# ray-project/rayfed

Hardware: AMD Instinct MI355X
Metric: cross_party_objects_per_sec (higher is better)
Workload: dtype int64; 1 GPU; model=many_tiny_tasks (2-party aggregate loop), global_batch=2576, seq_len=1, parallelism=fed2p-weak x1 lanes, transport=cpp

## Files before the change

### csrc/xfer_core.cpp

```cpp
#include <openssl/err.h>
#include <openssl/ssl.h>
#include <pybind11/functional.h>
#include <pybind11/pybind11.h>
#include <pybind11/stl.h>

#include <arpa/inet.h>
#include <netdb.h>
#include <netinet/in.h>
#include <netinet/tcp.h>
#include <sys/socket.h>
#include <sys/uio.h>
#include <unistd.h>

#include <atomic>
#include <condition_variable>
#include <cstring>
#include <deque>
#include <map>
#include <mutex>
#include <optional>
#include <stdexcept>
#include <string>
#include <thread>
#include <unordered_map>
#include <unordered_set>
#include <vector>

namespace py = pybind11;

namespace {

constexpr uint8_t kFlagDeferAck = 1;
constexpr uint8_t kFlagStripe = 2;
constexpr uint8_t kFlagPinned = 4;
constexpr const char* kPingSeqId = "ping";

extern "C" int hipHostMalloc(void** ptr, size_t size, unsigned int flags);
extern "C" int hipHostFree(void* ptr);

struct PinnedBuf {
  char* p = nullptr;
  size_t cap = 0;
  size_t len = 0;
  bool pinned = false;
  ~PinnedBuf();
};

class PinnedPool {
 public:
  static PinnedPool& inst() {
    static PinnedPool pool;
    return pool;
  }

  ~PinnedPool() {
    for (auto& [cls, bucket] : free_)
      for (auto& b : bucket) b->p = nullptr;
  }

  std::shared_ptr<PinnedBuf> acquire(size_t n) {
    size_t cls = 1ull << (64 - __builtin_clzll(std::max<size_t>(n, 1 << 16) - 1));
    {
      std::lock_guard<std::mutex> lk(mu_);
      auto& bucket = free_[cls];
      if (!bucket.empty()) {
        auto b = bucket.back();
        bucket.pop_back();
        b->len = n;
        return b;
      }
    }
    auto b = std::make_shared<PinnedBuf>();
    void* p = nullptr;
    if (hipHostMalloc(&p, cls, 0) == 0 && p) {
      b->p = (char*)p;
      b->pinned = true;
    } else {
      b->p = (char*)malloc(cls);
      if (!b->p) throw std::bad_alloc();
      b->pinned = false;
    }
    b->cap = cls;
    b->len = n;
    return b;
  }

  void release(std::shared_ptr<PinnedBuf> b) {
    std::lock_guard<std::mutex> lk(mu_);
    auto& bucket = free_[b->cap];
    size_t limit = b->cap >= (64u << 20) ? 16 : 8;
    if (bucket.size() < limit) bucket.push_back(std::move(b));
  }

 private:
  std::mutex mu_;
  std::unordered_map<size_t, std::vector<std::shared_ptr<PinnedBuf>>> free_;
};

PinnedBuf::~PinnedBuf() {
  if (!p) return;
  if (pinned)
    hipHostFree(p);
  else
    free(p);
}

static void write_all(int fd, const char* data, size_t n) {
  while (n) {
    ssize_t w = ::send(fd, data, n, MSG_NOSIGNAL);
    if (w < 0) {
      if (errno == EINTR) continue;
      throw std::runtime_error(std::string("send: ") + strerror(errno));
    }
    data += w;
    n -= (size_t)w;
  }
}

static void writev_all(int fd, std::vector<iovec> iov) {
  size_t idx = 0;
  while (idx < iov.size()) {
    ssize_t w = ::writev(fd, iov.data() + idx, (int)(iov.size() - idx));
    if (w < 0) {
      if (errno == EINTR) continue;
      throw std::runtime_error(std::string("writev: ") + strerror(errno));
    }
    size_t ww = (size_t)w;
    while (idx < iov.size() && ww >= iov[idx].iov_len) {
      ww -= iov[idx].iov_len;
      ++idx;
    }
    if (idx < iov.size() && ww) {
      iov[idx].iov_base = (char*)iov[idx].iov_base + ww;
      iov[idx].iov_len -= ww;
    }
  }
}

static bool read_all(int fd, char* data, size_t n) {
  while (n) {
    ssize_t r = ::recv(fd, data, n, 0);
    if (r < 0) {
      if (errno == EINTR) continue;
      return false;
    }
    if (r == 0) return false;
    data += r;
    n -= (size_t)r;
  }
  return true;
}

static void set_sock_opts(int fd) {
  int one = 1;
  setsockopt(fd, IPPROTO_TCP, TCP_NODELAY, &one, sizeof(one));
  int buf = 8 << 20;
  setsockopt(fd, SOL_SOCKET, SO_SNDBUF, &buf, sizeof(buf));
  setsockopt(fd, SOL_SOCKET, SO_RCVBUF, &buf, sizeof(buf));
}

static int spin_us() {
  static int v = [] {
    const char* e = getenv("RAYFED_SPIN_US");
    return e ? atoi(e) : 120;
  }();
  return v;
}

static std::string ssl_err() {
  char buf[256];
  ERR_error_string_n(ERR_get_error(), buf, sizeof(buf));
  return std::string(buf);
}

struct Stream {
  int fd = -1;
  SSL* ssl = nullptr;

  bool read_all(char* data, size_t n) {
    if (!ssl) return ::read_all(fd, data, n);
    while (n) {
      int r = SSL_read(ssl, data, (int)std::min(n, (size_t)1 << 20));
      if (r <= 0) return false;
      data += r;
      n -= (size_t)r;
    }
    return true;
// ... 23 lines not shown
      ::close(fd);
      fd = -1;
    }
  }
};

static SSL_CTX* make_server_ctx(const std::string& cert, const std::string& key,
                                const std::string& ca) {
  SSL_CTX* ctx = SSL_CTX_new(TLS_server_method());
  if (!ctx) throw std::runtime_error("SSL_CTX_new failed");
  SSL_CTX_set_min_proto_version(ctx, TLS1_2_VERSION);
  if (SSL_CTX_use_certificate_chain_file(ctx, cert.c_str()) != 1 ||
      SSL_CTX_use_PrivateKey_file(ctx, key.c_str(), SSL_FILETYPE_PEM) != 1) {
    SSL_CTX_free(ctx);
    throw std::runtime_error("server cert/key load failed: " + ssl_err());
  }
  if (!ca.empty()) {
    if (SSL_CTX_load_verify_locations(ctx, ca.c_str(), nullptr) != 1) {
      SSL_CTX_free(ctx);
      throw std::runtime_error("server CA load failed: " + ssl_err());
    }
    SSL_CTX_set_verify(
        ctx, SSL_VERIFY_PEER | SSL_VERIFY_FAIL_IF_NO_PEER_CERT, nullptr);
  }
  return ctx;
}

static SSL_CTX* make_client_ctx(const std::string& ca, const std::string& cert,
                                const std::string& key) {
  SSL_CTX* ctx = SSL_CTX_new(TLS_client_method());
  if (!ctx) throw std::runtime_error("SSL_CTX_new failed");
  SSL_CTX_set_min_proto_version(ctx, TLS1_2_VERSION);
  if (!ca.empty() && SSL_CTX_load_verify_locations(ctx, ca.c_str(), nullptr) != 1) {
    SSL_CTX_free(ctx);
    throw std::runtime_error("client CA load failed: " + ssl_err());
  }
  SSL_CTX_set_verify(ctx, SSL_VERIFY_PEER, nullptr);
  if (!cert.empty() && !key.empty()) {
    if (SSL_CTX_use_certificate_chain_file(ctx, cert.c_str()) != 1 ||
        SSL_CTX_use_PrivateKey_file(ctx, key.c_str(), SSL_FILETYPE_PEM) != 1) {
      SSL_CTX_free(ctx);
      throw std::runtime_error("client cert/key load failed: " + ssl_err());
    }
  }
  return ctx;
}

class BodyView {
 public:
  explicit BodyView(std::shared_ptr<PinnedBuf> b) : buf_(std::move(b)) {}
  ~BodyView() {
    if (buf_) {
      try {
        PinnedPool::inst().release(std::move(buf_));
      } catch (...) {
      }
    }
  }
  char* data() const { return buf_->p; }
  size_t size() const { return buf_->len; }
  bool pinned() const { return buf_->pinned; }

 private:
  std::shared_ptr<PinnedBuf> buf_;
};

class XferServer {
 public:
  XferServer(int port, std::string job_name, std::string tls_cert = "",
             std::string tls_key = "", std::string tls_ca = "")
      : job_(std::move(job_name)), port_(port) {
    if (!tls_cert.empty()) {
      ssl_ctx_ = make_server_ctx(tls_cert, tls_key, tls_ca);
    }
  }

  ~XferServer() {
    stop();
    if (ssl_ctx_) SSL_CTX_free(ssl_ctx_);
  }

  void start(py::object consume_cb) {
    consume_cb_ = std::move(consume_cb);
    listen_fd_ = ::socket(AF_INET, SOCK_STREAM, 0);
    if (listen_fd_ < 0) throw std::runtime_error("socket() failed");
    int zero = 0, one = 1;
    setsockopt(listen_fd_, SOL_SOCKET, SO_REUSEPORT, &zero, sizeof(zero));
    setsockopt(listen_fd_, SOL_SOCKET, SO_REUSEADDR, &one, sizeof(one));
    sockaddr_in addr{};
    addr.sin_family = AF_INET;
    addr.sin_addr.s_addr = htonl(INADDR_ANY);
    addr.sin_port = htons((uint16_t)port_);
    if (bind(listen_fd_, (sockaddr*)&addr, sizeof(addr)) != 0) {
      ::close(listen_fd_);
      listen_fd_ = -1;
      throw std::runtime_error("bind failed: port in use");
    }
    if (listen(listen_fd_, 64) != 0) {
      ::close(listen_fd_);
      listen_fd_ = -1;
      throw std::runtime_error("listen failed");
    }
    running_ = true;
    accept_thread_ = std::thread([this] { accept_loop(); });
  }

  void stop() {
    bool expected = true;
    if (!running_.compare_exchange_strong(expected, false)) return;
    ::shutdown(listen_fd_, SHUT_RDWR);
    ::close(listen_fd_);
    {
      std::lock_guard<std::mutex> lk(conn_mu_);
      for (auto& c : conns_) ::shutdown(c->st.fd, SHUT_RDWR);
    }
    if (accept_thread_.joinable()) accept_thread_.join();
    {
      std::lock_guard<std::mutex> lk(conn_mu_);
      for (auto& t : conn_threads_)
        if (t.joinable()) t.join();
      conn_threads_.clear();
    }
    {
      std::lock_guard<std::mutex> lk(tok_mu_);
      tokens_.clear();
    }
    std::lock_guard<std::mutex> lk(mail_mu_);
    stopped_ = true;
    pinned_mail_.clear();
    mail_cv_.notify_all();
  }

  void complete(uint64_t token, int code, const std::string& result) {
    std::shared_ptr<SrvConn> conn;
    uint64_t req_id = 0;
    {
      std::lock_guard<std::mutex> lk(tok_mu_);
      auto it = tokens_.find(token);
      if (it == tokens_.end()) return;
      conn = it->second.first;
      req_id = it->second.second;
      tokens_.erase(it);
    }
    if (!conn->alive.load()) return;
    try {
      write_ack(*conn, req_id, (uint16_t)code, result);
    } catch (...) {
      conn->alive = false;
      ::shutdown(conn->st.fd, SHUT_RDWR);
    }
  }

  py::bytes get_data(const std::string& up, const std::string& down,
                     double timeout_s) {
    std::string key = up + '\x00' + down;
    std::string body;
    {
      py::gil_scoped_release release;
      auto deadline = std::chrono::steady_clock::now() +
                      std::chrono::duration<double>(timeout_s);
      const auto spin_until = std::chrono::steady_clock::now() +
                              std::chrono::microseconds(spin_us());
      bool got = false;
      while (!got && std::chrono::steady_clock::now() < spin_until) {
        {
          std::unique_lock<std::mutex> lk(mail_mu_, std::try_to_lock);
          if (lk.owns_lock()) {
            auto it = mail_.find(key);
            if (it != mail_.end()) {
              body = std::move(it->second);
              mail_.erase(it);
              got = true;
              break;
            }
            if (stopped_) throw std::runtime_error("server stopped");
          }
        }
        for (int i = 0; i < 32; ++i) __builtin_ia32_pause();
      }
      if (!got) {
        std::unique_lock<std::mutex> lk(mail_mu_);
        while (true) {
          auto it = mail_.find(key);
          if (it != mail_.end()) {
            body = std::move(it->second);
            mail_.erase(it);
            break;
          }
          if (stopped_) throw std::runtime_error("server stopped");
          if (mail_cv_.wait_until(lk, deadline) == std::cv_status::timeout)
            throw std::runtime_error("get_data timeout");
        }
      }
    }
    return py::bytes(body);
  }

  void post(const std::string& up, const std::string& down,
            const std::string& body) {
    std::lock_guard<std::mutex> lk(mail_mu_);
    mail_[up + '\x00' + down] = body;
    mail_cv_.notify_all();
  }

  py::object wait_view(const std::string& up, const std::string& down,
                       double timeout_s) {
    std::string key = up + '\x00' + down;
    std::shared_ptr<PinnedBuf> b;
    {
      py::gil_scoped_release release;
      std::unique_lock<std::mutex> lk(mail_mu_);
      auto deadline = std::chrono::steady_clock::now() +
                      std::chrono::duration<double>(timeout_s);
      while (true) {
        auto it = pinned_mail_.find(key);
        if (it != pinned_mail_.end()) {
          b = std::move(it->second);
          pinned_mail_.erase(it);
          break;
        }
        if (stopped_) throw std::runtime_error("server stopped");
        if (mail_cv_.wait_until(lk, deadline) == std::cv_status::timeout)
          throw std::runtime_error("wait_view timeout");
      }
    }
    return py::cast(new BodyView(std::move(b)),
                    py::return_value_policy::take_ownership);
  }

  py::object try_view(const std::string& up, const std::string& down) {
    std::string key = up + '\x00' + down;
    std::shared_ptr<PinnedBuf> b;
    {
      std::lock_guard<std::mutex> lk(mail_mu_);
      auto it = pinned_mail_.find(key);
      if (it == pinned_mail_.end()) return py::none();
      b = std::move(it->second);
      pinned_mail_.erase(it);
    }
    return py::cast(new BodyView(std::move(b)),
                    py::return_value_policy::take_ownership);
  }

  std::optional<py::bytes> try_take(const std::string& up,
                                    const std::string& down) {
    std::string key = up + '\x00' + down;
    std::string body;
    {
      py::gil_scoped_release release;
      std::lock_guard<std::mutex> lk(mail_mu_);
      auto it = mail_.find(key);
      if (it == mail_.end()) return std::nullopt;
      body = std::move(it->second);
      mail_.erase(it);
    }
    return py::bytes(body);
  }

  uint64_t received_op_count() const { return recv_count_.load(); }

 private:
  struct SrvConn {
    Stream st;
    std::mutex write_mu;
    std::atomic<bool> alive{true};
  };

  struct Assembly {
    std::string data;
    std::shared_ptr<PinnedBuf> pbuf;
    std::atomic<uint64_t> got{0};
    uint64_t total;
    uint32_t cnt;
    std::unique_ptr<std::atomic<uint8_t>[]> seen;
    Assembly(uint64_t t, uint32_t c, bool pinned)
        : total(t), cnt(c), seen(new std::atomic<uint8_t>[c]) {
      for (uint32_t i = 0; i < c; ++i) seen[i].store(0);
      if (pinned)
        pbuf = PinnedPool::inst().acquire(t);
      else
        data.resize(t);
    }
    char* base() { return pbuf ? pbuf->p : data.data(); }
  };

  static bool drain(Stream& st, uint64_t n) {
    char scratch[65536];
    while (n) {
      size_t k = (size_t)std::min<uint64_t>(n, sizeof(scratch));
      if (!st.read_all(scratch, k)) return false;
      n -= k;
    }
    return true;
  }

  static void write_ack(SrvConn& c, uint64_t req_id, uint16_t code,
                        const std::string& result) {
    char ack[14];
    uint32_t ack_len = 10 + (uint32_t)result.size();
    memcpy(ack, &ack_len, 4);
    memcpy(ack + 4, &req_id, 8);
    memcpy(ack + 12, &code, 2);
    std::lock_guard<std::mutex> lk(c.write_mu);
    if (!c.alive.load()) throw std::runtime_error("connection closed");
    c.st.write_all(ack, 14);
    if (!result.empty()) c.st.write_all(result.data(), result.size());
  }

  void accept_loop() {
    while (running_) {
      int fd = ::accept(listen_fd_, nullptr, nullptr);
      if (fd < 0) {
        if (running_ && errno == EINTR) continue;
        break;
      }
      set_sock_opts(fd);
      auto conn = std::make_shared<SrvConn>();
      conn->st.fd = fd;
      std::lock_guard<std::mutex> lk(conn_mu_);
      conns_.push_back(conn);
      conn_threads_.emplace_back([this, conn] { conn_loop(conn); });
    }
  }

  void conn_loop(std::shared_ptr<SrvConn> conn) {
    Stream& st = conn->st;
    if (ssl_ctx_) {
      st.ssl = SSL_new(ssl_ctx_);
      SSL_set_fd(st.ssl, st.fd);
      if (SSL_accept(st.ssl) != 1) {
        conn->alive = false;
        st.close_free();
        return;
      }
    }
    std::vector<char> buf;
    while (running_) {
      char head[16];
      if (!st.read_all(head, 16)) break;
      uint64_t total, req_id;
      memcpy(&total, head, 8);
      memcpy(&req_id, head + 8, 8);
      if (total < 12 || total > (64ull << 30)) break;
      char meta[4];
      if (!st.read_all(meta, 4)) break;
      const uint8_t flags = (uint8_t)meta[0];
      const uint8_t job_len = (uint8_t)meta[1];
      const uint8_t up_len = (uint8_t)meta[2];
      const uint8_t down_len = (uint8_t)meta[3];
      const size_t names_len = (size_t)job_len + up_len + down_len;
      const size_t fixed =
          8 + 4 + names_len + ((flags & kFlagStripe) ? 24u : 0u);
      if (total < fixed) break;
      char names[768];
      if (!st.read_all(names, names_len)) break;
      std::string job(names, job_len);
      std::string up(names + job_len, up_len);
      std::string down(names + job_len + up_len, down_len);
      const uint64_t payload_len = total - fixed;

      uint16_t code = 200;
      std::string result = "OK";
      if (flags & kFlagStripe) {
        char smeta[24];
        if (!st.read_all(smeta, 24)) break;
        uint32_t idx, cnt;
        uint64_t s_off, body_total;
        memcpy(&idx, smeta, 4);
        memcpy(&cnt, smeta + 4, 4);
        memcpy(&s_off, smeta + 8, 8);
        memcpy(&body_total, smeta + 16, 8);
        if (cnt == 0 || idx >= cnt || body_total > (64ull << 30) ||
            s_off + payload_len > body_total)
          break;
        if (job != job_) {
          if (!drain(st, payload_len)) break;
          code = 417;
          result = "JobName mis-match: expected " + job_ + ", got " + job;
        } else {
          std::string key = up + '\x00' + down;
          const bool pinned = (flags & kFlagPinned) != 0;
          std::shared_ptr<Assembly> asmb;
          bool tombstoned = false;
          {
            std::lock_guard<std::mutex> lk(asm_mu_);
            auto& slot = asm_[key];
            if (!slot) {
              if (delivered_set_.count(key)) {
                asm_.erase(key);
                tombstoned = true;
              } else {
                slot = std::make_shared<Assembly>(body_total, cnt, pinned);
              }
            } else if (slot->total != body_total || slot->cnt != cnt) {
              slot = std::make_shared<Assembly>(body_total, cnt, pinned);
            }
            if (!tombstoned) asmb = slot;
          }
          if (tombstoned || asmb->seen[idx].exchange(1)) {
            if (!drain(st, payload_len)) break;
          } else
          if (!st.read_all(asmb->base() + s_off, payload_len)) {
            asmb->seen[idx].store(0);
            break;
          } else if (asmb->got.fetch_add(payload_len) + payload_len ==
                     body_total) {
            {
              std::lock_guard<std::mutex> lk(asm_mu_);
              asm_.erase(key);
              delivered_set_.insert(key);
              delivered_fifo_.push_back(key);
              if (delivered_fifo_.size() > 256) {
                delivered_set_.erase(delivered_fifo_.front());
                delivered_fifo_.pop_front();
              }
            }
            recv_count_.fetch_add(1);
            std::lock_guard<std::mutex> lk(mail_mu_);
            if (asmb->pbuf)
              pinned_mail_[key] = std::move(asmb->pbuf);
            else
              mail_[key] = std::move(asmb->data);
            mail_cv_.notify_all();
          }
        }
        try {
          write_ack(*conn, req_id, code, result);
        } catch (...) {
          break;
        }
        continue;
      }
      buf.resize(payload_len);
      if (!st.read_all(buf.data(), payload_len)) break;
      size_t off = 0;

      if (job != job_) {
        code = 417;
        result = "JobName mis-match: expected " + job_ + ", got " + job;
      } else if (up == kPingSeqId && down == kPingSeqId) {
      } else if (flags & kFlagDeferAck) {
        uint64_t token = next_token_.fetch_add(1);
        {
          std::lock_guard<std::mutex> lk(tok_mu_);
          tokens_[token] = {conn, req_id};
        }
        bool handed_off = false;
        {
          py::gil_scoped_acquire gil;
          try {
            py::bytes body(buf.data() + off, buf.size() - off);
            consume_cb_(up, down, body, token);
            handed_off = true;
          } catch (const std::exception& e) {
            code = 500;
            result = std::string("consume dispatch failed: ") + e.what();
          }
        }
        if (handed_off) continue;
        std::lock_guard<std::mutex> lk(tok_mu_);
        tokens_.erase(token);
      } else {
        recv_count_.fetch_add(1);
        std::lock_guard<std::mutex> lk(mail_mu_);
        mail_[up + '\x00' + down] =
            std::string(buf.data() + off, buf.size() - off);
        mail_cv_.notify_all();
      }

      try {
        write_ack(*conn, req_id, code, result);
      } catch (...) {
        break;
      }
    }
    {
      std::lock_guard<std::mutex> lk(conn->write_mu);
      conn->alive = false;
      st.close_free();
    }
  }

  std::string job_;
  int port_;
  int listen_fd_ = -1;
  std::atomic<bool> running_{false};
  bool stopped_ = false;
  std::thread accept_thread_;
  std::mutex conn_mu_;
  std::vector<std::shared_ptr<SrvConn>> conns_;
  std::vector<std::thread> conn_threads_;
  std::mutex mail_mu_;
  std::condition_variable mail_cv_;
  std::map<std::string, std::string> mail_;
  std::mutex asm_mu_;
  std::unordered_map<std::string, std::shared_ptr<Assembly>> asm_;
  std::unordered_set<std::string> delivered_set_;
  std::deque<std::string> delivered_fifo_;
  std::unordered_map<std::string, std::shared_ptr<PinnedBuf>> pinned_mail_;
  std::atomic<uint64_t> recv_count_{0};
  std::mutex tok_mu_;
  std::unordered_map<uint64_t, std::pair<std::shared_ptr<SrvConn>, uint64_t>>
      tokens_;
  std::atomic<uint64_t> next_token_{1};
  py::object consume_cb_;
  SSL_CTX* ssl_ctx_ = nullptr;
};

class XferClient {
 public:
  XferClient(std::string job_name, std::string tls_ca = "",
             std::string tls_cert = "", std::string tls_key = "",
             std::string server_name = "")
      : job_(std::move(job_name)), server_name_(std::move(server_name)) {
    if (!tls_ca.empty() || !tls_cert.empty()) {
      ssl_ctx_ = make_client_ctx(tls_ca, tls_cert, tls_key);
    }
  }
  ~XferClient() {
    close_all();
    if (ssl_ctx_) SSL_CTX_free(ssl_ctx_);
  }

  static std::vector<std::pair<const char*, size_t>> slice_views(
      const std::vector<std::pair<const char*, size_t>>& views, uint64_t lo,
      uint64_t hi) {
    std::vector<std::pair<const char*, size_t>> out;
    uint64_t pos = 0;
    for (const auto& v : views) {
      uint64_t vlo = pos, vhi = pos + v.second;
      pos = vhi;
      if (vhi <= lo || vlo >= hi) continue;
      uint64_t s = std::max(vlo, lo), e = std::min(vhi, hi);
      out.emplace_back(v.first + (s - vlo), (size_t)(e - s));
    }
    return out;
  }

  int send_striped(const std::string& host, int port, const std::string& up,
                   const std::string& down,
                   const std::vector<std::pair<const char*, size_t>>& views,
                   uint64_t body_len, int stripes, double timeout_s,
                   std::string* result_out, bool pinned = false) {
    std::string names;
    names.push_back((char)(kFlagStripe | (pinned ? kFlagPinned : 0)));
    names.push_back((char)job_.size());
    names.push_back((char)up.size());
    names.push_back((char)down.size());
    names += job_;
    names += up;
    names += down;
    const uint64_t chunk = (body_len + stripes - 1) / stripes;
    std::vector<int> codes((size_t)stripes, 0);
    std::vector<std::string> results((size_t)stripes);
    std::vector<std::string> errs((size_t)stripes);
    std::vector<std::thread> threads;
    for (int i = 0; i < stripes; ++i) {
      threads.emplace_back([&, i] {
        try {
          const uint64_t lo = (uint64_t)i * chunk;
          const uint64_t hi = std::min(body_len, lo + chunk);
          auto sub = slice_views(views, lo, hi);
          char smeta[24];
          uint32_t idx = (uint32_t)i, cnt = (uint32_t)stripes;
          memcpy(smeta, &idx, 4);
          memcpy(smeta + 4, &cnt, 4);
          memcpy(smeta + 8, &lo, 8);
          memcpy(smeta + 16, &body_len, 8);
          uint64_t total = 8 + names.size() + 24 + (hi - lo);
          if (ssl_ctx_) {
            codes[i] = stripe_tls(host, port, names, smeta, sub, total,
                                  timeout_s, &results[i]);
            return;
          }
          std::shared_ptr<Conn> conn_sp = get_conn(host, port, i + 1);
          Conn& conn = *conn_sp;
          std::shared_ptr<Pending> pending = std::make_shared<Pending>();
          uint64_t req_id;
          {
            std::lock_guard<std::mutex> lk(conn.write_mu);
            req_id = conn.next_id++;
            {
              std::lock_guard<std::mutex> lk2(conn.pend_mu);
              conn.pending[req_id] = pending;
            }
            char head[16];
            memcpy(head, &total, 8);
            memcpy(head + 8, &req_id, 8);
            std::vector<iovec> iov;
            iov.push_back({head, 16});
            iov.push_back({(void*)names.data(), names.size()});
            iov.push_back({smeta, 24});
            for (auto& v : sub) iov.push_back({(void*)v.first, v.second});
            try {
              writev_all(conn.fd, std::move(iov));
            } catch (...) {
              conn.alive = false;
              throw;
            }
          }
          std::unique_lock<std::mutex> lk(pending->mu);
          auto deadline = std::chrono::steady_clock::now() +
                          std::chrono::duration<double>(timeout_s);
          while (!pending->done) {
            if (pending->cv.wait_until(lk, deadline) ==
                std::cv_status::timeout)
              throw std::runtime_error("stripe ack timeout");
          }
          if (pending->broken)
            throw std::runtime_error("connection broken awaiting stripe ack");
          codes[i] = pending->code;
          results[i] = pending->result;
        } catch (const std::exception& e) {
          errs[i] = e.what();
        }
      });
    }
    for (auto& t : threads) t.join();
    for (int i = 0; i < stripes; ++i)
      if (!errs[i].empty())
        throw std::runtime_error("stripe " + std::to_string(i) +
                                 " failed: " + errs[i]);
    for (int i = 0; i < stripes; ++i) {
      if (codes[i] != 200) {
        if (result_out) *result_out = results[i];
        return codes[i];
      }
    }
    if (result_out) *result_out = "OK";
    return 200;
  }

  int stripe_tls(const std::string& host, int port, const std::string& names,
                 const char* smeta,
                 const std::vector<std::pair<const char*, size_t>>& sub,
                 uint64_t total, double timeout_s, std::string* result_out) {
    std::string key = host + ":" + std::to_string(port);
    std::unique_ptr<Stream> st = acquire_tls_conn(key, host, port);
    set_recv_timeout(st->fd, std::max(1.0, timeout_s));
    uint64_t req_id = tls_req_id_.fetch_add(1);
    try {
      char head[16];
      memcpy(head, &total, 8);
      memcpy(head + 8, &req_id, 8);
      std::vector<iovec> iov;
      iov.push_back({head, 16});
      iov.push_back({(void*)names.data(), names.size()});
      iov.push_back({(void*)smeta, 24});
      for (auto& v : sub) iov.push_back({(void*)v.first, v.second});
      st->write_iov(std::move(iov));
      char ahead[14];
      if (!st->read_all(ahead, 14))
        throw std::runtime_error("connection broken awaiting stripe ack");
      uint32_t len;
      uint64_t rid;
      uint16_t code;
      memcpy(&len, ahead, 4);
      memcpy(&rid, ahead + 4, 8);
      memcpy(&code, ahead + 12, 2);
      std::string result;
      if (len > 10) {
        result.resize(len - 10);
        if (!st->read_all(result.data(), result.size()))
          throw std::runtime_error("connection broken reading stripe ack");
      }
      if (rid != req_id)
        throw std::runtime_error("ack id mismatch on TLS stripe");
      release_tls_conn(key, std::move(st));
      if (result_out) *result_out = result;
      return code;
    } catch (...) {
      st->close_free();
      throw;
    }
  }

  int send(const std::string& host, int port, const std::string& up,
           const std::string& down, std::vector<py::buffer> parts,
           bool defer_ack, double timeout_s, std::string* result_out,
           int stripes = 1, bool pinned = false) {
    std::vector<std::pair<const char*, size_t>> views;
    views.reserve(parts.size());
    size_t body_len = 0;
    std::vector<py::buffer_info> infos;
    infos.reserve(parts.size());
    for (auto& b : parts) {
      infos.emplace_back(b.request());
      auto& info = infos.back();
      views.emplace_back((const char*)info.ptr,
                         (size_t)(info.size * info.itemsize));
      body_len += views.back().second;
    }

    if (stripes > 1 && !defer_ack && body_len > 0) {
      py::gil_scoped_release release;
      return send_striped(host, port, up, down, views, body_len, stripes,
                          timeout_s, result_out, pinned);
    }

    uint8_t flags = defer_ack ? kFlagDeferAck : 0;
    std::string preamble;
    preamble.push_back((char)flags);
    preamble.push_back((char)job_.size());
    preamble.push_back((char)up.size());
    preamble.push_back((char)down.size());
    preamble += job_;
    preamble += up;
    preamble += down;

    uint64_t total = 8  + preamble.size() + body_len;

    int code;
    std::string result;
// ... 247 lines not shown
    std::unordered_map<std::string, std::shared_ptr<Conn>> conns;
    {
      std::lock_guard<std::mutex> lk(conns_mu_);
      conns.swap(conns_);
    }
    for (auto& [key, conn] : conns) {
      ::shutdown(conn->fd, SHUT_RDWR);
      if (conn->reader.joinable()) conn->reader.join();
      ::close(conn->fd);
    }
    std::lock_guard<std::mutex> lk2(tls_mu_);
    for (auto& [key, pool] : tls_pool_)
      for (auto& st : pool) st->close_free();
    tls_pool_.clear();
  }

 private:
  struct Pending {
    std::mutex mu;
    std::condition_variable cv;
    std::atomic<bool> done{false};
    bool broken = false;
    uint16_t code = 0;
    std::string result;
  };

  struct Conn {
    int fd = -1;
    uint64_t next_id = 1;
    std::mutex write_mu;
    std::mutex pend_mu;
    std::unordered_map<uint64_t, std::shared_ptr<Pending>> pending;
    std::thread reader;
    std::atomic<bool> alive{true};
  };

  std::shared_ptr<Conn> get_conn(const std::string& host, int port,
                                 int slot = 0) {
    std::string key = host + ":" + std::to_string(port);
    if (slot) key += "#" + std::to_string(slot);
    std::lock_guard<std::mutex> lk(conns_mu_);
    auto it = conns_.find(key);
    if (it != conns_.end() && it->second->alive) return it->second;
    int fd = ::socket(AF_INET, SOCK_STREAM, 0);
    if (fd < 0) throw std::runtime_error("socket() failed");
    sockaddr_in addr{};
    addr.sin_family = AF_INET;
    addr.sin_port = htons((uint16_t)port);
    if (inet_pton(AF_INET, host.c_str(), &addr.sin_addr) != 1) {
      hostent* he = gethostbyname(host.c_str());
      if (!he) {
        ::close(fd);
        throw std::runtime_error("resolve failed: " + host);
      }
      memcpy(&addr.sin_addr, he->h_addr, sizeof(addr.sin_addr));
    }
    if (connect(fd, (sockaddr*)&addr, sizeof(addr)) != 0) {
      ::close(fd);
      throw std::runtime_error(std::string("connect failed: ") +
                               strerror(errno));
    }
    set_sock_opts(fd);
    auto conn = std::make_shared<Conn>();
    conn->fd = fd;
    std::shared_ptr<Conn> sp = conn;
    conn->reader = std::thread([this, sp] { reader_loop(sp.get()); });
    auto& entry = conns_[key];
    if (entry) {
      ::shutdown(entry->fd, SHUT_RDWR);
      if (entry->reader.joinable()) entry->reader.detach();
      dead_.push_back(entry);
    }
    entry = conn;
    return conn;
  }

  void reader_loop(Conn* conn) {
    while (true) {
      char head[14];
      if (!read_all(conn->fd, head, 14)) break;
      uint32_t len;
      uint64_t req_id;
      uint16_t code;
      memcpy(&len, head, 4);
      memcpy(&req_id, head + 4, 8);
      memcpy(&code, head + 12, 2);
      std::string result;
      if (len > 10) {
        result.resize(len - 10);
        if (!read_all(conn->fd, result.data(), result.size())) break;
      }
      std::shared_ptr<Pending> p;
      {
        std::lock_guard<std::mutex> lk(conn->pend_mu);
        auto it = conn->pending.find(req_id);
        if (it != conn->pending.end()) {
          p = it->second;
          conn->pending.erase(it);
        }
      }
      if (p) {
        std::lock_guard<std::mutex> lk(p->mu);
        p->done = true;
        p->code = code;
        p->result = std::move(result);
        p->cv.notify_all();
      }
    }
    conn->alive = false;
    std::lock_guard<std::mutex> lk(conn->pend_mu);
    for (auto& [id, p] : conn->pending) {
      std::lock_guard<std::mutex> lk2(p->mu);
      p->done = true;
      p->broken = true;
      p->cv.notify_all();
    }
    conn->pending.clear();
  }

  std::string job_;
  std::string server_name_;
  SSL_CTX* ssl_ctx_ = nullptr;
  std::mutex conns_mu_;
  std::unordered_map<std::string, std::shared_ptr<Conn>> conns_;
  std::vector<std::shared_ptr<Conn>> dead_;
  std::mutex tls_mu_;
  std::unordered_map<std::string, std::vector<std::unique_ptr<Stream>>> tls_pool_;
  std::atomic<uint64_t> tls_req_id_{1};
  std::mutex async_mu_;
  std::unordered_map<uint64_t, std::shared_ptr<Pending>> async_;
  std::atomic<uint64_t> async_id_{1};
};

}

PYBIND11_MODULE(_xfer, m) {
  m.doc() = "rayfed_amd C++ transport core (plaintext cross-silo hot path)";
  py::class_<BodyView>(m, "BodyView", py::buffer_protocol())
      .def_buffer([](BodyView& v) {
        return py::buffer_info(v.data(), sizeof(uint8_t),
                               py::format_descriptor<uint8_t>::format(), 1,
                               {v.size()}, {sizeof(uint8_t)});
      })
      .def("__len__", &BodyView::size)
      .def_property_readonly("pinned", &BodyView::pinned);
  py::class_<XferServer>(m, "XferServer")
      .def(py::init<int, std::string, std::string, std::string, std::string>(),
           py::arg("port"), py::arg("job_name"), py::arg("tls_cert") = "",
           py::arg("tls_key") = "", py::arg("tls_ca") = "")
      .def("start", &XferServer::start, py::arg("consume_cb"))
      .def("stop", &XferServer::stop,
           py::call_guard<py::gil_scoped_release>())
      .def("get_data", &XferServer::get_data, py::arg("up"), py::arg("down"),
           py::arg("timeout_s") = 600.0)
      .def("complete", &XferServer::complete, py::arg("token"),
           py::arg("code"), py::arg("result") = std::string(),
           py::call_guard<py::gil_scoped_release>())
      .def("post", &XferServer::post, py::call_guard<py::gil_scoped_release>())
      .def("wait_view", &XferServer::wait_view, py::arg("up"),
           py::arg("down"), py::arg("timeout_s") = 60.0)
      .def("try_view", &XferServer::try_view)
      .def("try_take", &XferServer::try_take)
      .def_property_readonly("received_op_count",
                             &XferServer::received_op_count);
  py::class_<XferClient>(m, "XferClient")
      .def(py::init<std::string, std::string, std::string, std::string,
                    std::string>(),
           py::arg("job_name"), py::arg("tls_ca") = "",
           py::arg("tls_cert") = "", py::arg("tls_key") = "",
           py::arg("server_name") = "")
      .def(
          "send",
          [](XferClient& c, const std::string& host, int port,
             const std::string& up, const std::string& down,
             std::vector<py::buffer> parts, bool defer_ack,
             double timeout_s, int stripes, bool pinned) {
            std::string result;
            int code =
                c.send(host, port, up, down, std::move(parts), defer_ack,
                       timeout_s, &result, stripes, pinned);
            return py::make_tuple(code, result);
          },
          py::arg("host"), py::arg("port"), py::arg("up"), py::arg("down"),
          py::arg("parts"), py::arg("defer_ack") = false,
          py::arg("timeout_s") = 60.0, py::arg("stripes") = 1,
          py::arg("pinned") = false)
      .def("send_async", &XferClient::send_async, py::arg("host"),
           py::arg("port"), py::arg("up"), py::arg("down"), py::arg("parts"),
           py::arg("defer_ack") = false)
      .def("wait_ack", &XferClient::wait_ack, py::arg("handle"),
           py::arg("timeout_s") = 60.0,
           py::call_guard<py::gil_scoped_release>())
      .def("close_all", &XferClient::close_all,
           py::call_guard<py::gil_scoped_release>());
}
```

### rayfed_amd/proxy/xfer.py

```python
from __future__ import annotations

import logging
import threading
import time
from concurrent.futures import Future, ThreadPoolExecutor
from concurrent.futures import TimeoutError as FutureTimeoutError
from typing import Dict, Optional

from rayfed_amd import config as fed_config
from rayfed_amd.ops import tensor_codec
from rayfed_amd.proxy.grpc import frames
from rayfed_amd.runtime.object_ref import ObjectRef

logger = logging.getLogger(__name__)

_OBJ_MARKER = b"\x00RFOBJ"


def _load_xfer():
    import torch

    import rayfed_amd._xfer as xfer

    return xfer
# ... 558 lines not shown
        self.gpu_plane = None
        self._stats_lock = threading.Lock()
        self.receive_op_count = 0
        self._deferred_count = 0

    @property
    def proxy(self):
        return self

    @property
    def received_op_count(self) -> int:
        return int(self._server.received_op_count) + self._deferred_count

    def _consume_deferred(self, up: str, down: str, body: bytes, token: int):
        self._consume_pool.submit(self._consume_one, up, down, body, token)

    def _consume_one(self, up: str, down: str, body: bytes, token: int):
        try:
            kind, header, payload = frames.decode_frame(body)
            obj = tensor_codec.decode(
                {k: header[k] for k in ("skel", "tensors", "ipc_group")
                 if k in header},
                memoryview(payload),
                self.gpu_plane,
                self._allowed_list,
                allow_lazy=True,
            )
        except Exception as e:
            logger.warning("xfer deferred consume failed: %r", e)
            self._server.complete(token, 500, f"consume failed: {e!r}")
            return
        lazies = (
            self.gpu_plane.pop_pending_lazies()
            if self.gpu_plane is not None
            else []
        )
        with self._objs_lock:
            self._objs[(up, down)] = obj
            self._deferred_count += 1
        self._server.post(up, down, _OBJ_MARKER)
        if not lazies:
            self._server.complete(token, 200)
            return
        remaining = [len(lazies)]
        lock = threading.Lock()

        def _one_done():
            with lock:
                remaining[0] -= 1
                done = remaining[0] == 0
            if done:
                self._server.complete(token, 200)

        for lz in lazies:
            lz._attach_completer(_one_done)

    def _take(self, up: str, down: str, body: bytes):
        if bytes(body) == _OBJ_MARKER:
            with self._objs_lock:
                return self._objs.pop((up, down))
        kind, header, payload = frames.decode_frame(body)
        from rayfed_amd._private import serialization

        if kind == frames.KIND_ERROR:
            raise serialization.loads(payload, self._allowed_list)
        if kind == frames.KIND_TENSOR:
            return tensor_codec.decode(
                header, memoryview(payload), self.gpu_plane, self._allowed_list
            )
        if kind == frames.KIND_CHUNKED:
            _ik, inner_header, _ = frames.decode_frame(payload)
            return tensor_codec.decode_streamed(
                inner_header, header["xlen"], header["xc"],
                self._iter_chunks(up, down, header["xk"]),
                self.gpu_plane, self._allowed_list,
            )
        return serialization.loads(payload, self._allowed_list)

    def _iter_chunks(self, up: str, down: str, k: int):
        import time as _time

        remaining = set(range(k))
        deadline = _time.monotonic() + 600
        while remaining:
            got = None
            for i in sorted(remaining):
                b = self._server.try_view(f"{up}\x01x{i}", down)
                if b is not None:
                    got = (i, b)
                    break
            if got is None:
                err = self._server.try_take(up, down)
                if err is not None:
                    self._take(up, down, err)
                    raise RuntimeError(
                        "unexpected non-error frame during chunked receive"
                    )
                if _time.monotonic() > deadline:
                    raise TimeoutError("chunk-streamed receive stalled")
                i = min(remaining)
                try:
                    b = self._server.wait_view(f"{up}\x01x{i}", down, 0.25)
                    got = (i, b)
                except RuntimeError as e:
                    if "timeout" in str(e):
                        continue
                    raise
            remaining.discard(got[0])
            if _xfer_debug():
                import sys as _sys

                print(f"[xfer-rx] chunk {got[0]} ({len(got[1])>>20}MiB) "
                      f"t={_time.monotonic():.3f}",
                      file=_sys.stderr, flush=True)
            yield got

    def get_data(self, src_party, upstream_seq_id, curr_seq_id) -> Future:
        up, down = str(upstream_seq_id), str(curr_seq_id)
        with self._stats_lock:
            self.receive_op_count += 1
        body = self._server.try_take(up, down)
        if body is not None:
            fut: Future = Future()
            try:
                fut.set_result(self._take(up, down, body))
            except BaseException as e:
                fut.set_exception(e)
            return fut

        def _wait(timeout=None):
            deadline = None if timeout is None else time.monotonic() + timeout
            while True:
                if deadline is None:
                    chunk = 60.0
                else:
                    chunk = min(60.0, deadline - time.monotonic())
                    if chunk <= 0:
                        raise FutureTimeoutError()
                try:
                    b = self._server.get_data(up, down, chunk)
                    break
                except RuntimeError as e:
                    if "timeout" in str(e):
                        continue
                    raise
            return self._take(up, down, b)

        return _LazyFuture(_wait)

    def _get_stats(self) -> Dict[str, int]:
        return {"receive_op_count": self.receive_op_count}

    def stop(self):
        self._server.stop()
        self._pool.shutdown(wait=False, cancel_futures=True)
        self._consume_pool.shutdown(wait=False, cancel_futures=True)


class _LazyFuture(Future):

    def __init__(self, fetch):
        super().__init__()
        self._fetch = fetch
        self._claim = threading.Lock()

    def result(self, timeout=None):
        if not self.done() and self._claim.acquire(blocking=False):
            try:
                if not self.done():
                    try:
                        value = self._fetch(timeout)
                    except FutureTimeoutError:
                        raise
                    except BaseException as e:
                        self.set_exception(e)
                    else:
                        self.set_result(value)
            finally:
                self._claim.release()
        return super().result(timeout)

    def exception(self, timeout=None):
        if not self.done():
            try:
                self.result(timeout)
            except BaseException:
                pass
        return super().exception(timeout)
```

### setup.py

```python
import os

from setuptools import find_packages, setup

os.environ.setdefault("PYTORCH_ROCM_ARCH", "gfx950")

from torch.utils import cpp_extension

setup(
    name="rayfed_amd",
    version="0.2.0",
    packages=find_packages(include=["rayfed_amd", "rayfed_amd.*"]),
    ext_modules=[
        cpp_extension.CUDAExtension(
            name="rayfed_amd._hip",
            sources=["csrc/rayfed_hip.hip"],
            include_dirs=[os.path.abspath("csrc")],
            extra_compile_args={
                "cxx": ["-O3", "-std=c++17"],
                "nvcc": ["-O3", "-std=c++17"],
            },
        ),
        cpp_extension.CppExtension(
            name="rayfed_amd._xfer",
            sources=["csrc/xfer_core.cpp"],
            extra_compile_args=["-O3", "-std=c++17", "-pthread"],
            libraries=["ssl", "crypto", "amdhip64"],
            library_dirs=["/opt/rocm/lib"],
            include_dirs=["/opt/rocm/include"],
        ),
    ],
    cmdclass={"build_ext": cpp_extension.BuildExtension},
)
```

Measured before the change: 15220 objects/s.

## Let spinning receivers pump small frames directly from connection sockets

While get_data spins waiting for a message, the waiting thread now peeks each plain (non-TLS) connection socket and consumes small unflagged frames itself, delivering its own payload directly and posting others to the mailbox. This removes the cross-thread handoff from the connection thread to the waiter through the mutex and condition variable. Connection threads now poll and take a per-connection rx mutex so the two readers never interleave on one socket. Acks are also coalesced into a single write, and stripe chunking is guarded for small bodies. The change adds locking complexity and extra recv syscalls per spin iteration.

```diff
diff --git a/csrc/xfer_core.cpp b/csrc/xfer_core.cpp
--- a/csrc/xfer_core.cpp
+++ b/csrc/xfer_core.cpp
@@ -8,6 +8,7 @@
 #include <netdb.h>
 #include <netinet/in.h>
 #include <netinet/tcp.h>
+#include <poll.h>
 #include <sys/socket.h>
 #include <sys/uio.h>
 #include <unistd.h>
@@ -26,13 +27,15 @@
 #include <unordered_set>
 #include <vector>
 
+#include "xfer_rx.h"
+
 namespace py = pybind11;
 
 namespace {
 
-constexpr uint8_t kFlagDeferAck = 1;
-constexpr uint8_t kFlagStripe = 2;
-constexpr uint8_t kFlagPinned = 4;
+using xfer_rx::kFlagDeferAck;
+using xfer_rx::kFlagStripe;
+using xfer_rx::kFlagPinned;
 constexpr const char* kPingSeqId = "ping";
 
 extern "C" int hipHostMalloc(void** ptr, size_t size, unsigned int flags);
@@ -362,16 +365,25 @@
   }
 
   py::bytes get_data(const std::string& up, const std::string& down,
-                     double timeout_s) {
+                     double timeout_s, int spin_us_arg = -1) {
     std::string key = up + '\x00' + down;
     std::string body;
     {
       py::gil_scoped_release release;
-      auto deadline = std::chrono::steady_clock::now() +
-                      std::chrono::duration<double>(timeout_s);
-      const auto spin_until = std::chrono::steady_clock::now() +
-                              std::chrono::microseconds(spin_us());
+      const auto start = std::chrono::steady_clock::now();
+      auto deadline = start + std::chrono::duration<double>(timeout_s);
+      const int spin = spin_us_arg < 0 ? spin_us() : spin_us_arg;
+      const auto spin_until =
+          std::min<std::chrono::steady_clock::time_point>(
+              start + std::chrono::microseconds(spin),
+              std::chrono::time_point_cast<
+                  std::chrono::steady_clock::duration>(deadline));
       bool got = false;
+      const bool pump = spin > 0 && !ssl_ctx_;
+      std::vector<std::shared_ptr<SrvConn>> snap;
+      std::vector<uint8_t> backoff;
+      uint64_t snap_gen = 0;
+      bool have_snap = false;
       while (!got && std::chrono::steady_clock::now() < spin_until) {
         {
           std::unique_lock<std::mutex> lk(mail_mu_, std::try_to_lock);
@@ -386,10 +398,36 @@
             if (stopped_) throw std::runtime_error("server stopped");
           }
         }
+        if (pump) {
+          const uint64_t gen = conn_gen_.load(std::memory_order_acquire);
+          if (!have_snap || gen != snap_gen) {
+            snap.clear();
+            std::lock_guard<std::mutex> lk(conn_mu_);
+            snap_gen = conn_gen_.load(std::memory_order_acquire);
+            for (auto& c : conns_)
+              if (c->alive.load()) snap.push_back(c);
+            backoff.assign(snap.size(), 0);
+            have_snap = true;
+          }
+          for (size_t ci = 0; ci < snap.size(); ++ci) {
+            if (backoff[ci]) {
+              --backoff[ci];
+              continue;
+            }
+            bool left = false;
+            if (pump_conn(*snap[ci], key, &body, &left)) {
+              got = true;
+              break;
+            }
+            if (left) backoff[ci] = 64;
+          }
+          if (got) break;
+        }
         for (int i = 0; i < 32; ++i) __builtin_ia32_pause();
       }
       if (!got) {
         std::unique_lock<std::mutex> lk(mail_mu_);
+        bool parked = false;
         while (true) {
           auto it = mail_.find(key);
           if (it != mail_.end()) {
@@ -398,6 +436,10 @@
             break;
           }
           if (stopped_) throw std::runtime_error("server stopped");
+          if (!parked) {
+            parked = true;
+            rx_parked_.fetch_add(1, std::memory_order_relaxed);
+          }
           if (mail_cv_.wait_until(lk, deadline) == std::cv_status::timeout)
             throw std::runtime_error("get_data timeout");
         }
@@ -469,9 +511,18 @@
 
   uint64_t received_op_count() const { return recv_count_.load(); }
 
+  py::dict rx_stats() const {
+    py::dict d;
+    d["waiter"] = rx_waiter_.load();
+    d["conn"] = rx_conn_.load();
+    d["parked"] = rx_parked_.load();
+    return d;
+  }
+
  private:
   struct SrvConn {
     Stream st;
+    std::mutex rx_mu;
     std::mutex write_mu;
     std::atomic<bool> alive{true};
   };
@@ -511,10 +562,65 @@
     memcpy(ack, &ack_len, 4);
     memcpy(ack + 4, &req_id, 8);
     memcpy(ack + 12, &code, 2);
+    char small[14 + 64];
+    std::string big;
+    char* out = small;
+    if (result.size() > sizeof(small) - 14) {
+      big.resize(14 + result.size());
+      out = big.data();
+    }
+    memcpy(out, ack, 14);
+    memcpy(out + 14, result.data(), result.size());
     std::lock_guard<std::mutex> lk(c.write_mu);
     if (!c.alive.load()) throw std::runtime_error("connection closed");
-    c.st.write_all(ack, 14);
-    if (!result.empty()) c.st.write_all(result.data(), result.size());
+    c.st.write_all(out, 14 + result.size());
+  }
+
+  bool pump_conn(SrvConn& c, const std::string& want_key,
+                 std::string* body_out, bool* left) {
+    if (!c.alive.load(std::memory_order_relaxed)) return false;
+    char buf[xfer_rx::kSmallFrameMax];
+    xfer_rx::Preamble pre;
+    {
+      std::unique_lock<std::mutex> rx(c.rx_mu, std::try_to_lock);
+      if (!rx.owns_lock() || !c.alive.load()) return false;
+      const xfer_rx::Took took =
+          xfer_rx::take_small_frame(c.st.fd, job_, buf, sizeof(buf), &pre);
+      if (took != xfer_rx::Took::kFrame) {
+        *left = took == xfer_rx::Took::kLeft;
+        return false;
+      }
+    }
+    const char* names = buf + xfer_rx::Preamble::names_off();
+    std::string key;
+    key.reserve((size_t)pre.up_len + 1 + pre.down_len);
+    key.append(names + pre.job_len, pre.up_len);
+    key.push_back('\x00');
+    key.append(names + pre.job_len + pre.up_len, pre.down_len);
+    const char* body = buf + pre.body_off();
+    const size_t body_len = (size_t)pre.payload_len;
+    bool mine = false;
+    if (pre.up_len == 4 && pre.down_len == 4 &&
+        memcmp(names + pre.job_len, "pingping", 8) == 0) {
+    } else {
+      recv_count_.fetch_add(1);
+      rx_waiter_.fetch_add(1, std::memory_order_relaxed);
+      if (key == want_key) {
+        body_out->assign(body, body_len);
+        mine = true;
+      } else {
+        std::lock_guard<std::mutex> lk(mail_mu_);
+        mail_[key] = std::string(body, body_len);
+        mail_cv_.notify_all();
+      }
+    }
+    try {
+      write_ack(c, pre.req_id, 200, "OK");
+    } catch (...) {
+      std::lock_guard<std::mutex> rx(c.rx_mu);
+      if (c.alive.load()) ::shutdown(c.st.fd, SHUT_RDWR);
+    }
+    return mine;
   }
 
   void accept_loop() {
@@ -530,6 +636,7 @@
       std::lock_guard<std::mutex> lk(conn_mu_);
       conns_.push_back(conn);
       conn_threads_.emplace_back([this, conn] { conn_loop(conn); });
+      conn_gen_.fetch_add(1, std::memory_order_release);
     }
   }
 
@@ -544,30 +651,39 @@
         return;
       }
     }
+    const bool plain = st.ssl == nullptr;
     std::vector<char> buf;
     while (running_) {
-      char head[16];
-      if (!st.read_all(head, 16)) break;
-      uint64_t total, req_id;
-      memcpy(&total, head, 8);
-      memcpy(&req_id, head + 8, 8);
-      if (total < 12 || total > (64ull << 30)) break;
-      char meta[4];
-      if (!st.read_all(meta, 4)) break;
-      const uint8_t flags = (uint8_t)meta[0];
-      const uint8_t job_len = (uint8_t)meta[1];
-      const uint8_t up_len = (uint8_t)meta[2];
-      const uint8_t down_len = (uint8_t)meta[3];
-      const size_t names_len = (size_t)job_len + up_len + down_len;
-      const size_t fixed =
-          8 + 4 + names_len + ((flags & kFlagStripe) ? 24u : 0u);
-      if (total < fixed) break;
-      char names[768];
-      if (!st.read_all(names, names_len)) break;
-      std::string job(names, job_len);
-      std::string up(names + job_len, up_len);
-      std::string down(names + job_len + up_len, down_len);
-      const uint64_t payload_len = total - fixed;
+      char hm[xfer_rx::kHeadMetaLen];
+      std::unique_lock<std::mutex> rx(conn->rx_mu, std::defer_lock);
+      if (plain) {
+        pollfd pfd{st.fd, POLLIN, 0};
+        int pr = ::poll(&pfd, 1, 500);
+        if (pr < 0 && errno != EINTR) break;
+        if (pr <= 0) continue;
+        rx.lock();
+        ssize_t r = ::recv(st.fd, hm, sizeof(hm), MSG_DONTWAIT);
+        if (r < 0) {
+          if (errno == EAGAIN || errno == EWOULDBLOCK || errno == EINTR)
+            continue;
+          break;
+        }
+        if (r == 0) break;
+        if ((size_t)r < sizeof(hm) &&
+            !st.read_all(hm + r, sizeof(hm) - (size_t)r))
+          break;
+      } else {
+        if (!st.read_all(hm, sizeof(hm))) break;
+      }
+      xfer_rx::Preamble pre;
+      if (!xfer_rx::parse_head_meta(hm, &pre)) break;
+      const uint64_t req_id = pre.req_id;
+      const uint8_t flags = pre.flags;
+      char names[xfer_rx::kMaxNamesLen];
+      if (!st.read_all(names, pre.names_len)) break;
+      std::string job, up, down;
+      xfer_rx::split_names(pre, names, &job, &up, &down);
+      const uint64_t payload_len = pre.payload_len;
 
       uint16_t code = 200;
       std::string result = "OK";
@@ -626,6 +742,7 @@
               }
             }
             recv_count_.fetch_add(1);
+            rx_conn_.fetch_add(1, std::memory_order_relaxed);
             std::lock_guard<std::mutex> lk(mail_mu_);
             if (asmb->pbuf)
               pinned_mail_[key] = std::move(asmb->pbuf);
@@ -634,6 +751,7 @@
             mail_cv_.notify_all();
           }
         }
+        if (rx.owns_lock()) rx.unlock();
         try {
           write_ack(*conn, req_id, code, result);
         } catch (...) {
@@ -656,6 +774,7 @@
           tokens_[token] = {conn, req_id};
         }
         bool handed_off = false;
+        if (rx.owns_lock()) rx.unlock();
         {
           py::gil_scoped_acquire gil;
           try {
@@ -672,12 +791,14 @@
         tokens_.erase(token);
       } else {
         recv_count_.fetch_add(1);
+        rx_conn_.fetch_add(1, std::memory_order_relaxed);
         std::lock_guard<std::mutex> lk(mail_mu_);
         mail_[up + '\x00' + down] =
             std::string(buf.data() + off, buf.size() - off);
         mail_cv_.notify_all();
       }
 
+      if (rx.owns_lock()) rx.unlock();
       try {
         write_ack(*conn, req_id, code, result);
       } catch (...) {
@@ -685,6 +806,7 @@
       }
     }
     {
+      std::lock_guard<std::mutex> rxl(conn->rx_mu);
       std::lock_guard<std::mutex> lk(conn->write_mu);
       conn->alive = false;
       st.close_free();
@@ -709,6 +831,10 @@
   std::deque<std::string> delivered_fifo_;
   std::unordered_map<std::string, std::shared_ptr<PinnedBuf>> pinned_mail_;
   std::atomic<uint64_t> recv_count_{0};
+  std::atomic<uint64_t> conn_gen_{0};
+  std::atomic<uint64_t> rx_waiter_{0};
+  std::atomic<uint64_t> rx_conn_{0};
+  std::atomic<uint64_t> rx_parked_{0};
   std::mutex tok_mu_;
   std::unordered_map<uint64_t, std::pair<std::shared_ptr<SrvConn>, uint64_t>>
       tokens_;
@@ -760,7 +886,9 @@
     names += job_;
     names += up;
     names += down;
-    const uint64_t chunk = (body_len + stripes - 1) / stripes;
+    const uint64_t chunk =
+        std::max<uint64_t>(1, (body_len + stripes - 1) / stripes);
+    stripes = (int)std::max<uint64_t>(1, (body_len + chunk - 1) / chunk);
     std::vector<int> codes((size_t)stripes, 0);
     std::vector<std::string> results((size_t)stripes);
     std::vector<std::string> errs((size_t)stripes);
@@ -768,7 +896,7 @@
     for (int i = 0; i < stripes; ++i) {
       threads.emplace_back([&, i] {
         try {
-          const uint64_t lo = (uint64_t)i * chunk;
+          const uint64_t lo = std::min(body_len, (uint64_t)i * chunk);
           const uint64_t hi = std::min(body_len, lo + chunk);
           auto sub = slice_views(views, lo, hi);
           char smeta[24];
@@ -1322,7 +1450,7 @@
       .def("stop", &XferServer::stop,
            py::call_guard<py::gil_scoped_release>())
       .def("get_data", &XferServer::get_data, py::arg("up"), py::arg("down"),
-           py::arg("timeout_s") = 600.0)
+           py::arg("timeout_s") = 600.0, py::arg("spin_us") = -1)
       .def("complete", &XferServer::complete, py::arg("token"),
            py::arg("code"), py::arg("result") = std::string(),
            py::call_guard<py::gil_scoped_release>())
@@ -1332,7 +1460,8 @@
       .def("try_view", &XferServer::try_view)
       .def("try_take", &XferServer::try_take)
       .def_property_readonly("received_op_count",
-                             &XferServer::received_op_count);
+                             &XferServer::received_op_count)
+      .def_property_readonly("rx_stats", &XferServer::rx_stats);
   py::class_<XferClient>(m, "XferClient")
       .def(py::init<std::string, std::string, std::string, std::string,
                     std::string>(),
diff --git a/csrc/xfer_rx.h b/csrc/xfer_rx.h
--- /dev/null
+++ b/csrc/xfer_rx.h
@@ -0,0 +1,125 @@
+#pragma once
+
+#include <sys/socket.h>
+#include <sys/types.h>
+
+#include <cerrno>
+#include <cstdint>
+#include <cstring>
+#include <string>
+
+namespace xfer_rx {
+
+constexpr uint8_t kFlagDeferAck = 1;
+constexpr uint8_t kFlagStripe = 2;
+constexpr uint8_t kFlagPinned = 4;
+
+constexpr size_t kHeadLen = 16;
+constexpr size_t kMetaLen = 4;
+constexpr size_t kHeadMetaLen = kHeadLen + kMetaLen;
+constexpr size_t kStripeMetaLen = 24;
+constexpr size_t kMaxNamesLen = 3 * 255;
+constexpr uint64_t kMaxTotal = 64ull << 30;
+constexpr size_t kSmallFrameMax = 64 * 1024;
+
+struct Preamble {
+  uint64_t total = 0;
+  uint64_t req_id = 0;
+  uint8_t flags = 0;
+  uint8_t job_len = 0;
+  uint8_t up_len = 0;
+  uint8_t down_len = 0;
+  size_t names_len = 0;
+  size_t fixed = 0;
+  uint64_t payload_len = 0;
+
+  uint64_t frame_len() const { return kHeadLen + (total - 8); }
+  static constexpr size_t names_off() { return kHeadMetaLen; }
+  size_t body_off() const { return kHeadMetaLen + names_len; }
+};
+
+inline bool parse_head_meta(const char* p, Preamble* out) {
+  Preamble pre;
+  memcpy(&pre.total, p, 8);
+  memcpy(&pre.req_id, p + 8, 8);
+  if (pre.total < 12 || pre.total > kMaxTotal) return false;
+  pre.flags = (uint8_t)p[16];
+  pre.job_len = (uint8_t)p[17];
+  pre.up_len = (uint8_t)p[18];
+  pre.down_len = (uint8_t)p[19];
+  pre.names_len = (size_t)pre.job_len + pre.up_len + pre.down_len;
+  pre.fixed = 8 + kMetaLen + pre.names_len +
+              ((pre.flags & kFlagStripe) ? kStripeMetaLen : 0u);
+  if (pre.total < pre.fixed) return false;
+  pre.payload_len = pre.total - pre.fixed;
+  *out = pre;
+  return true;
+}
+
+inline void split_names(const Preamble& pre, const char* names,
+                        std::string* job, std::string* up,
+                        std::string* down) {
+  job->assign(names, pre.job_len);
+  up->assign(names + pre.job_len, pre.up_len);
+  down->assign(names + pre.job_len + pre.up_len, pre.down_len);
+}
+
+enum class Peeked {
+  kIncomplete,
+  kPlainSmall,
+  kLeave,
+  kBad,
+};
+
+inline Peeked classify_peeked(const char* buf, size_t n,
+                              const std::string& job, Preamble* out) {
+  if (n < kHeadMetaLen) return Peeked::kIncomplete;
+  Preamble pre;
+  if (!parse_head_meta(buf, &pre)) return Peeked::kBad;
+  if (pre.flags != 0) return Peeked::kLeave;
+  if (pre.frame_len() > kSmallFrameMax) return Peeked::kLeave;
+  if (n < pre.frame_len()) return Peeked::kIncomplete;
+  if (pre.job_len != job.size() ||
+      memcmp(buf + Preamble::names_off(), job.data(), job.size()) != 0)
+    return Peeked::kLeave;
+  *out = pre;
+  return Peeked::kPlainSmall;
+}
+
+enum class Took {
+  kEmpty,
+  kFrame,
+  kIncomplete,
+  kLeft,
+};
+
+inline Took take_small_frame(int fd, const std::string& job, char* buf,
+                             size_t cap, Preamble* out) {
+  if (cap > kSmallFrameMax) cap = kSmallFrameMax;
+  ssize_t r;
+  do {
+    r = ::recv(fd, buf, cap, MSG_PEEK | MSG_DONTWAIT);
+  } while (r < 0 && errno == EINTR);
+  if (r < 0 && (errno == EAGAIN || errno == EWOULDBLOCK)) return Took::kEmpty;
+  if (r <= 0) return Took::kLeft;
+  Preamble pre;
+  switch (classify_peeked(buf, (size_t)r, job, &pre)) {
+    case Peeked::kPlainSmall:
+      break;
+    case Peeked::kIncomplete:
+      return (size_t)r >= cap ? Took::kLeft : Took::kIncomplete;
+    default:
+      return Took::kLeft;
+  }
+  size_t want = (size_t)pre.frame_len(), have = 0;
+  while (have < want) {
+    ssize_t t = ::recv(fd, buf + have, want - have, MSG_DONTWAIT);
+    if (t < 0 && errno == EINTR) continue;
+    if (t <= 0) return Took::kLeft;
+    have += (size_t)t;
+  }
+  *out = pre;
+  return Took::kFrame;
+}
+
+}
diff --git a/rayfed_amd/proxy/xfer.py b/rayfed_amd/proxy/xfer.py
--- a/rayfed_amd/proxy/xfer.py
+++ b/rayfed_amd/proxy/xfer.py
@@ -734,6 +734,15 @@
         return {"receive_op_count": self.receive_op_count}
 
     def stop(self):
+        import os
+
+        if os.environ.get("RAYFED_RX_STATS") == "1":
+            import sys as _sys
+
+            print(f"[xfer-rx] party={self._party} "
+                  f"rx_stats={dict(self._server.rx_stats)} "
+                  f"received={int(self._server.received_op_count)}",
+                  file=_sys.stderr, flush=True)
         self._server.stop()
         self._pool.shutdown(wait=False, cancel_futures=True)
         self._consume_pool.shutdown(wait=False, cancel_futures=True)
diff --git a/setup.py b/setup.py
--- a/setup.py
+++ b/setup.py
@@ -23,6 +23,7 @@
         cpp_extension.CppExtension(
             name="rayfed_amd._xfer",
             sources=["csrc/xfer_core.cpp"],
+            depends=["csrc/xfer_rx.h"],
             extra_compile_args=["-O3", "-std=c++17", "-pthread"],
             libraries=["ssl", "crypto", "amdhip64"],
             library_dirs=["/opt/rocm/lib"],
```

Measured after the change: 9713 objects/s. 0.638x the previous value.
